# ufcg-lsd/custom-k8s-scheduler

Measured on AMD Instinct MI355X. Metric: pods scheduled/sec (exact sequential stream, 5,000 nodes x 100,000 pods), higher is better.
Workload: dtype int32+f64; 1 GPU; config2: 5,000 nodes x 100,000 pods, exact sequential, Fit+Balanced+QoS weights, percentageOfNodesToScore=100; engine=lookahead, launch=resident, table_layout=compact, lookahead=32, parallelism=single

## Files before the change

### custom-k8s-scheduler_amd/csrc/qs_ctx.hpp

```cpp
#pragma once
#include <hip/hip_runtime.h>
#include <rccl/rccl.h>

#include <mutex>
#include <string>
#include <vector>

#include "../../include/qsched.h"
#include "qs_device.hpp"
#include "qs_launch.hpp"

namespace qs_host {

constexpr int64_t kLimit = (1LL << 24) - 1;
constexpr int64_t kWideMemLimit = (1LL << 46) - 1;
constexpr int64_t kGrowLimit32 = (1LL << 31) - 1;
constexpr int64_t kGrowLimitF64 = (1LL << 53) - 1;
constexpr uint32_t kSoaMinNodes = 1u << 16;
constexpr uint32_t kAaMaxNodes = 1u << 20;

struct QsError {
    qs_status st;
    std::string msg;
};
// ... 66 lines not shown
    uint64_t epoch_after = 0;
    int shift = 0;
    bool wide = false;
    qs_ctx *owner = nullptr;
    hipGraphExec_t gexec = nullptr;
    std::vector<uint8_t> gkey;
    ~qs_stream() {
        if (gexec) (void)hipGraphExecDestroy(gexec);
    }
};

struct qs_ctx {
    std::mutex mu;
    uint64_t table_epoch = 0;
    qs_config cfg{};
    int device = 0;
    hipStream_t stream = nullptr;
    hipStream_t stream2 = nullptr;
    std::string err;
    qs_host::Mirror m;
    int shift = 20;
    bool wide = false;
    bool dev_valid = false;
    uint32_t zero_alloc = 0;
    qs::DevTable dt{};
    qs::DevCfg dc{};
    int32_t strat = 0;
    qs_host::DevBuf strat_tab;
    std::vector<qs_stream *> streams;
    qs_host::DevBuf tbl;
    qs_host::DevBuf soa;
    bool soa_valid = false;
    qs_host::DevBuf tbl_saved;
    qs_host::Mirror m_saved;
    bool saved = false;
    bool saved_wide = false;
    int saved_shift = 20;
    bool mirror_stale = false;
    uint64_t device_faults = 0;
    qs_host::DevBuf diag;
    qs_host::DevBuf scratch, lists, clists, dio, npart, normi, nstat, nfall, nrec, bctrl, one_pod, one_podx;
    qs_host::DevBuf vshard;
    void *pin = nullptr;
    size_t pin_bytes = 0;
    uint64_t score_seq = 0;
    qs_host::DevBuf score_gs;
    uint32_t pend = 0xFFFFFFFFu;
    qs_host::DevBuf hand;
    bool handoff_off = false;
    qs_host::DevBuf resctl;
    int res_timeouts = 0;
    bool res_cooldown = false;
    uint32_t inject_used = 0;
    bool last_resident = false;
    int32_t last_res_path = 0;
    int cus = 0;
    uint64_t run_seq = 0;
    bool last_waits = false;
    uint32_t cap = 0;
    int rank = 0, world = 1;
    ncclComm_t comm = nullptr;
    qs_host::DevBuf mbox, mbox_peers;
    std::vector<void *> mbox_opened;
    bool mbox_on = false;
    bool mbox_fine = false;
    bool mbox_broken = false;
    bool mbox_host = false;
    void *mbox_hptr = nullptr;
    std::string mbox_shm;
    std::vector<void *> mbox_hmaps;
};
namespace qs_host {
void mbox_host_release(qs_ctx *c);
}

namespace qs_host {
struct ShardPlan {
    uint32_t W, v0, nv;
};
inline ShardPlan shard_plan(const qs_ctx *c) {
    if (c->world > 1) return {(uint32_t)c->world, (uint32_t)c->rank, 1u};
    if (c->cfg.virtual_shards > 1) return {(uint32_t)c->cfg.virtual_shards, 0u, (uint32_t)c->cfg.virtual_shards};
    return {1u, 0u, 1u};
}
void exchange_lists(qs_ctx *c, uint64_t *lists, size_t per_rank_entries, hipStream_t stream);
void exchange_u32(qs_ctx *c, uint32_t *buf, size_t per_rank_words, hipStream_t stream);
void allreduce_max_u64(qs_ctx *c, uint64_t *buf, size_t count, hipStream_t stream);
void allreduce_max_u32(qs_ctx *c, uint32_t *buf, size_t count, hipStream_t stream);
constexpr size_t kDioWords = 68;
constexpr size_t kMbRanks = 16, kMbSlots = 3, kMbPartPerRank = 4096;
constexpr size_t kMbFlags = 2 * kMbRanks * 8;
constexpr size_t kMbListSlot = kMbRanks * 64 * 64 * 8;
constexpr size_t kMbPartSlot = kMbRanks * kMbPartPerRank * 16;
constexpr size_t kMbResSlots = 4, kMbResPods = 32;
constexpr size_t kMbResHello = kMbFlags + kMbSlots * (kMbListSlot + kMbPartSlot);
constexpr size_t kMbResFlags = kMbResHello + 256;
constexpr size_t kMbResLists = kMbResFlags + kMbResSlots * kMbResPods * kMbRanks * 8;
constexpr size_t kMbResNFlags = kMbResLists + kMbResSlots * kMbResPods * kMbRanks * 64 * 8;
constexpr size_t kMbResNorm = kMbResNFlags + kMbResSlots * kMbResPods * kMbRanks * 8;
constexpr size_t kMbBytes = kMbResNorm + kMbResSlots * kMbResPods * kMbRanks * 16;
inline uint64_t *mbox_lists(qs_ctx *c, uint32_t slot) {
    return reinterpret_cast<uint64_t *>(static_cast<char *>(c->mbox.p) + kMbFlags + slot * kMbListSlot);
}
inline uint4 *mbox_npart(qs_ctx *c, uint32_t slot) {
    return reinterpret_cast<uint4 *>(static_cast<char *>(c->mbox.p) + kMbFlags + kMbSlots * kMbListSlot +
                                     slot * kMbPartSlot);
// ... 6 lines not shown
```

### custom-k8s-scheduler_amd/csrc/qs_host.cpp

```cpp
#include "../../include/qsched.h"

#include <hip/hip_runtime.h>

#include <algorithm>
#include <atomic>
#include <chrono>
#include <cmath>
#include <cstddef>
#include <cstdio>
#include <cstdlib>
#include <cstring>
#include <exception>
#include <mutex>
#include <new>
#include <string>
#include <vector>
#include <functional>
#include <condition_variable>
#include <thread>

#include "qs_ctx.hpp"

using namespace qs;

using namespace qs_host;

namespace {

uint32_t feat_of(const qs_config &c) {
    uint32_t f = 0;
    if (c.enable_taint) f |= kFeatTaint;
    if (c.enable_affinity) f |= kFeatAffinity;
    return f;
}

void check_cfg(const qs_config &c) {
    if (c.abi_version != QS_ABI_VERSION) fail(QS_EINVAL, "qs_config.abi_version mismatch");
    if (c.fit_weight_cpu < 0 || c.fit_weight_mem < 0 || c.fit_weight_cpu > 65535 ||
        c.fit_weight_mem > 65535)
        fail(QS_EINVAL, "fit weights out of range");
    int64_t wmax = 0;
    for (int q = 0; q < 3; q++) {
        if (c.w_fit[q] < 0 || c.w_bal[q] < 0 || c.w_fit[q] > 65535 || c.w_bal[q] > 65535)
            fail(QS_EINVAL, "plugin weights must be in [0, 65535]");
        wmax = std::max<int64_t>(wmax, (int64_t)c.w_fit[q] + c.w_bal[q]);
    }
    if (c.w_taint < 0 || c.w_affinity < 0 || c.w_taint > 65535 || c.w_affinity > 65535)
        fail(QS_EINVAL, "plugin weights must be in [0, 65535]");
    if (c.n_fit_resources < 0 || c.n_fit_resources > QS_MAX_SCORE_RES)
        fail(QS_EINVAL, "n_fit_resources must be in [0, 4]");
    if (c.n_balanced_resources < 0 || c.n_balanced_resources > QS_MAX_SCORE_RES)
        fail(QS_EINVAL, "n_balanced_resources must be in [0, 4]");
    uint32_t seen = 0;
    for (int i = 0; i < c.n_fit_resources; i++) {
        const int32_t r = c.fit_resources[i].resource;
        if (r < QS_RES_CPU || r > QS_RES_EXT1) fail(QS_EINVAL, "fit_resources: unknown resource");
        if (seen & (1u << r)) fail(QS_EINVAL, "fit_resources: duplicate resource");
        seen |= 1u << r;
        if (c.fit_resources[i].weight < 1 || c.fit_resources[i].weight > 100)
            fail(QS_EINVAL, "fit_resources: weight must be in [1, 100]");
    }
    seen = 0;
    for (int i = 0; i < c.n_balanced_resources; i++) {
        const int32_t r = c.balanced_resources[i];
        if (r < QS_RES_CPU || r > QS_RES_EXT1) fail(QS_EINVAL, "balanced_resources: unknown resource");
        if (seen & (1u << r)) fail(QS_EINVAL, "balanced_resources: duplicate resource");
        seen |= 1u << r;
    }
    const int64_t tmax = 100 * (wmax + (c.enable_taint ? c.w_taint : 0) +
                                (c.enable_affinity ? c.w_affinity : 0));
    if (tmax >= 0x7FFFFFFF) fail(QS_EINVAL, "weighted total would overflow the packed key");
}

void fit_weights(const qs_config &c, int64_t w[5]) {
    for (int r = 0; r < 5; r++) w[r] = 0;
    if (c.n_fit_resources == 0) {
        w[QS_RES_CPU] = c.fit_weight_cpu;
        w[QS_RES_MEMORY] = c.fit_weight_mem;
        return;
    }
// ... 193 lines not shown
    for (uint32_t i = 0; i < n; i++) {
        const HostRow r = compact_row(c->m, i, c->shift, wide);
        if (wide) wrows[i] = to_drow_wide(r);
        else rows[i] = to_drow(r);
        masks[i] = DMask{r.th, r.ts, r.lb0, r.lb1};
        if (soa) {
            const int32_t f[kSCols] = {r.ac, r.am, r.rc, r.rm, r.zc, r.zm, r.np, r.mp, r.ae0, r.re0, r.ae1, r.re1};
            for (int k = 0; k < kSCols; k++) cols[(size_t)k * c->cap + i] = f[k];
        }
    }
    if (n) {
        if (wide) HIPCHK(hipMemcpyAsync(c->dt.wrows, wrows.data(), n * sizeof(DRowW), hipMemcpyHostToDevice, c->stream));
        else HIPCHK(hipMemcpyAsync(c->dt.rows, rows.data(), n * sizeof(DRow), hipMemcpyHostToDevice, c->stream));
        HIPCHK(hipMemcpyAsync(c->dt.masks, masks.data(), n * sizeof(DMask), hipMemcpyHostToDevice, c->stream));
        HIPCHK(hipMemcpyAsync(c->dt.zone, c->m.zone.data(), n * 4, hipMemcpyHostToDevice, c->stream));
    }
    if (c->dt.apps) {
        HIPCHK(hipMemsetAsync(c->dt.apps, 0, (size_t)kAppWords * c->cap * 4, c->stream));
        HIPCHK(hipMemsetAsync(c->dt.zcount, 0, (size_t)kMaxApps * kMaxZones * 4, c->stream));
    }
    if (soa) {
        c->soa.ensure(cols.size() * 4);
        for (int k = 0; k < kSCols; k++) c->dt.soa.c[k] = c->soa.as<int32_t>() + (size_t)k * c->cap;
        HIPCHK(hipMemcpyAsync(c->soa.p, cols.data(), cols.size() * 4, hipMemcpyHostToDevice, c->stream));
    }
    HIPCHK(hipStreamSynchronize(c->stream));
    c->dev_valid = true;
    c->soa_valid = soa;
    c->mirror_stale = false;
}

void ensure_soa(qs_ctx *c) {
    if (!c->dt.soa.c[0] || c->soa_valid) return;
    HIPCHK(launch_rows_to_soa(c->dt, c->stream));
    c->soa_valid = true;
}

void push_row(qs_ctx *c, uint32_t i, bool sync = true) {
    if (!c->dev_valid) return;
    const HostRow r = compact_row(c->m, i, c->shift, c->wide);
    hipLaunchKernelGGL(k_set_row, dim3(1), dim3(1), 0, c->stream, c->dt, i, r,
                       kFeatExt | kFeatTaint | kFeatAffinity);
    HIPCHK(hipGetLastError());
    if (sync) HIPCHK(hipStreamSynchronize(c->stream));
}

void flush_pending(qs_ctx *c) {
    if (c->pend == 0xFFFFFFFFu) return;
    const uint32_t i = c->pend;
    c->pend = 0xFFFFFFFFu;
    if (c->dev_valid && i < c->m.n) push_row(c, i, false);
}

void sync_mirror(qs_ctx *c) {
    if (!c->mirror_stale || !c->dev_valid) return;
    const uint32_t n = c->m.n;
    Mirror &m = c->m;
    if (c->wide) {
        std::vector<DRowW> rows(n);
        if (n) HIPCHK(hipMemcpyAsync(rows.data(), c->dt.wrows, n * sizeof(DRowW), hipMemcpyDeviceToHost, c->stream));
        HIPCHK(hipStreamSynchronize(c->stream));
        for (uint32_t i = 0; i < n; i++) {
            m.rc[i] = rows[i].rc;
            m.rm[i] = (int64_t)rows[i].rm;
            m.zc[i] = rows[i].zc;
            m.zm[i] = (int64_t)rows[i].zm;
            m.np[i] = rows[i].np;
            m.re[(size_t)i * QS_MAX_EXT] = rows[i].re0;
            m.re[(size_t)i * QS_MAX_EXT + 1] = rows[i].re1;
        }
    } else {
        std::vector<DRow> rows(n);
        if (n) HIPCHK(hipMemcpyAsync(rows.data(), c->dt.rows, n * sizeof(DRow), hipMemcpyDeviceToHost, c->stream));
        HIPCHK(hipStreamSynchronize(c->stream));
        for (uint32_t i = 0; i < n; i++) {
            m.rc[i] = rows[i].rc;
            m.rm[i] = (int64_t)rows[i].rm << c->shift;
            m.zc[i] = rows[i].zc;
            m.zm[i] = (int64_t)rows[i].zm << c->shift;
            m.np[i] = rows[i].np;
            m.re[(size_t)i * QS_MAX_EXT] = rows[i].re0;
            m.re[(size_t)i * QS_MAX_EXT + 1] = rows[i].re1;
        }
    }
    c->mirror_stale = false;
}

int pod_min_shift(const qs_pod &p) { return std::min(ctz64(p.req_mem), ctz64(p.nz_mem)); }

void check_pod(const qs_pod &p, uint32_t j) {
    auto bad = [&](const char *w) {
        fail(QS_EINVAL, std::string("pod ") + std::to_string(j) + ": " + w);
    };
    if (p.qos < 0 || p.qos > 2) bad("qos must be 0..2");
    if (p.req_cpu < 0 || p.req_mem < 0 || p.nz_cpu < 0 || p.nz_mem < 0) bad("negative request");
    for (int k = 0; k < QS_MAX_EXT; k++)
        if (p.req_ext[k] < 0 || p.req_ext[k] > kLimit) bad("req_ext out of range");
    if (p.req_cpu > kLimit || p.nz_cpu > kLimit) bad("cpu request out of range");
    if (p.req_mem > kWideMemLimit || p.nz_mem > kWideMemLimit) bad("memory request above 2^46 bytes");
    if (p.n_req_terms < 0 || p.n_req_terms > QS_MAX_TERMS || p.n_pref_terms < 0 ||
        p.n_pref_terms > QS_MAX_TERMS)
        bad("term count out of range");
    for (int t = 0; t < p.n_pref_terms; t++)
        if (p.pref_weight[t] < 0 || p.pref_weight[t] > 100) bad("preferred term weight must be 0..100");
    if (p.app < 0 || p.app >= QS_MAX_APPS) bad("app outside [0, QS_MAX_APPS)");
    if (p.anti_affinity < QS_AA_NONE || p.anti_affinity > QS_AA_ZONE) bad("anti_affinity must be 0..2");
}

uint32_t pod_flags(const qs_ctx *c, const qs_pod &p) {
    const uint32_t aff = c->cfg.enable_affinity ? 1u : 0u;
    return (uint32_t)p.qos | (aff * (uint32_t)p.n_req_terms << 4) | (aff * (uint32_t)p.n_pref_terms << 8) |
           ((uint32_t)p.anti_affinity << 12) | ((uint32_t)p.app << 16);
}

size_t pod_record_bytes(bool wide) { return wide ? sizeof(DPodW) : sizeof(DPod); }

void compact_pod(const qs_ctx *c, const qs_pod &p, uint32_t j, int shift, bool wide, void *dst) {
    check_pod(p, j);
    if (wide) {
        DPodW d{};
        d.rc = (int32_t)p.req_cpu;
        d.zc = (int32_t)p.nz_cpu;
        d.rm = (double)p.req_mem;
        d.zm = (double)p.nz_mem;
        d.re0 = (int32_t)p.req_ext[0];
        d.re1 = (int32_t)p.req_ext[1];
        d.wfit = (uint16_t)c->cfg.w_fit[p.qos];
// ... 362 lines not shown
    for (int q = 0; q < 3; q++) { cfg->w_fit[q] = wf[q]; cfg->w_bal[q] = wb[q]; }
    cfg->w_taint = 3;
    cfg->w_affinity = 2;
    cfg->qos_sort = 1;
}

qs_status qs_open(const qs_config *cfg, int device, qs_ctx **out) {
    g_open_err.clear();
    if (!cfg || !out) return open_failed(QS_EINVAL, "qs_open: null config or output pointer");
    *out = nullptr;
    qs_ctx *c = new (std::nothrow) qs_ctx();
    if (!c) return QS_ENOMEM;
    try {
        check_cfg(*cfg);
        c->cfg = *cfg;
        c->device = device;
        int ndev = 0;
        HIPCHK(hipGetDeviceCount(&ndev));
        if (device < 0 || device >= ndev) fail(QS_EINVAL, "no such device");
        HIPCHK(hipSetDevice(device));
        HIPCHK(hipStreamCreateWithFlags(&c->stream, hipStreamNonBlocking));
        HIPCHK(hipStreamCreateWithFlags(&c->stream2, hipStreamNonBlocking));
        c->dc = make_devcfg(c->cfg);
        c->scratch.ensure(scan_scratch_bytes());
        HIPCHK(hipMemset(c->scratch.p, 0, scan_scratch_bytes()));
    } catch (const QsError &e) {
        delete c;
        return open_failed(e.st, e.msg);
    } catch (...) {
        delete c;
        return open_failed(QS_EDEVICE, "qs_open: unexpected failure");
    }
    *out = c;
    return QS_OK;
}

qs_status qs_close(qs_ctx *c) {
    if (!c) return QS_EINVAL;
    {
        std::lock_guard<std::mutex> lk(c->mu);
        (void)hipSetDevice(c->device);
        if (c->stream) (void)hipStreamSynchronize(c->stream);
        if (c->comm) (void)ncclCommDestroy(c->comm);
        c->comm = nullptr;
        for (void *p : c->mbox_opened) (void)hipIpcCloseMemHandle(p);
        c->mbox_opened.clear();
        mbox_host_release(c);
        for (qs_stream *ps : c->streams) ps->owner = nullptr;
        c->streams.clear();
    }
    hipStream_t s = c->stream, s2 = c->stream2;
    if (s2) (void)hipStreamSynchronize(s2);
    if (c->pin) (void)hipHostFree(c->pin);
    delete c;
    if (s) (void)hipStreamDestroy(s);
    if (s2) (void)hipStreamDestroy(s2);
    return QS_OK;
}

static void shape_table(const qs_shape_point *sh, uint32_t n, uint8_t table[101]) {
    if (!sh || !table) fail(QS_EINVAL, "shape: null pointer");
    if (n < 1 || n > QS_MAX_SHAPE) fail(QS_EINVAL, "shape: 1 to 16 points");
    for (uint32_t i = 0; i < n; i++) {
        if (sh[i].utilization < 0 || sh[i].utilization > 100) fail(QS_EINVAL, "shape: utilization must be in [0, 100]");
        if (sh[i].score < 0 || sh[i].score > 10) fail(QS_EINVAL, "shape: score must be in [0, 10]");
        if (i && sh[i].utilization <= sh[i - 1].utilization)
            fail(QS_EINVAL, "shape: utilization must be strictly increasing");
    }
    for (int64_t p = 0; p <= 100; p++) {
        int64_t v = (int64_t)sh[n - 1].score * 10;
        for (uint32_t i = 0; i < n; i++) {
            if (p > sh[i].utilization) continue;
            const int64_t s1 = (int64_t)sh[i].score * 10;
            if (i == 0) { v = s1; break; }
            const int64_t s0 = (int64_t)sh[i - 1].score * 10, u0 = sh[i - 1].utilization, u1 = sh[i].utilization;
            v = s0 + (s1 - s0) * (p - u0) / (u1 - u0);
            break;
        }
        table[p] = (uint8_t)v;
    }
}

qs_status qs_shape_table(const qs_shape_point *shape, uint32_t n, uint8_t table[101]) {
    try {
        shape_table(shape, n, table);
    } catch (const QsError &) {
        return QS_EINVAL;
    }
    return QS_OK;
}

qs_status qs_set_scoring_strategy(qs_ctx *c, const qs_scoring_strategy *s) {
    return guarded(c, [&] {
        if (!s) fail(QS_EINVAL, "null scoring strategy");
        if (s->type != QS_STRATEGY_LEAST_ALLOCATED && s->type != QS_STRATEGY_MOST_ALLOCATED &&
            s->type != QS_STRATEGY_REQUESTED_TO_CAPACITY_RATIO)
            fail(QS_EINVAL, "unknown scoring strategy type");
        if (s->type != QS_STRATEGY_REQUESTED_TO_CAPACITY_RATIO && s->n_shape != 0)
            fail(QS_EINVAL, "a shape is given for a scoring strategy that takes none");
        alignas(16) uint8_t tab[128] = {0};
        if (s->type == QS_STRATEGY_REQUESTED_TO_CAPACITY_RATIO) {
            if (s->n_shape < 1 || s->n_shape > QS_MAX_SHAPE) fail(QS_EINVAL, "shape: 1 to 16 points");
            shape_table(s->shape, (uint32_t)s->n_shape, tab);
        } else {
            for (int p = 0; p <= 100; p++) tab[p] = (uint8_t)p;
        }
// ... 389 lines not shown
        if (g_sdiag && pk) score_diag_report(c->score_seq, std::chrono::steady_clock::now());
    }, true);
}

qs_status qs_stream_prepare(qs_ctx *c, const qs_pod *pods, uint32_t p, qs_stream **out) {
    if (!out) return QS_EINVAL;
    *out = nullptr;
    qs_stream *s = nullptr;
    qs_status st = guarded(c, [&] {
        if (p && !pods) fail(QS_EINVAL, "null pods");
        HIPCHK(hipSetDevice(c->device));
        s = new qs_stream();
        s->p = p;
        s->pods.assign(pods, pods + p);
        for (uint32_t j = 0; j < p; j++) check_pod(pods[j], j);
        ensure_layout(c, pods, p);
        s->shift = c->shift;
        s->wide = c->wide;
        s->feat = feat_of(c->cfg) | (c->wide ? kFeatWide | kFeatExt : 0u);
        bool has_ext = false;
        for (uint32_t j = 0; j < p && !has_ext; j++) has_ext = pods[j].req_ext[0] || pods[j].req_ext[1];
        if (has_ext) s->feat |= kFeatExt;
        s->feat |= res_feat(c->cfg, has_ext) | strat_feat(c);
        s->order = qos_order(pods, p, c->cfg.qos_sort != 0);
        const size_t rb = pod_record_bytes(c->wide);
        std::vector<uint8_t> dp(rb * std::max<uint32_t>(p, 1));
        const bool needx = feat_of(c->cfg) & (kFeatTaint | kFeatAffinity);
        std::vector<DPodX> dx(needx ? std::max<uint32_t>(p, 1) : 1);
        for (uint32_t k = 0; k < p; k++) {
            const uint32_t j = s->order[k];
            compact_pod(c, pods[j], j, c->shift, c->wide, dp.data() + rb * k);
            if (needx) dx[k] = compact_podx(c, pods[j]);
        }
        const size_t P1 = std::max<uint32_t>(p, 1);
        s->d_pods.ensure(rb * P1);
        s->d_podx.ensure(sizeof(DPodX) * dx.size());
        s->d_node.ensure(4 * P1);
        s->d_key.ensure(8 * P1);
        if (c->cfg.record_timestamps) s->d_stamp.ensure(8 * P1);
        HIPCHK(hipMemcpyAsync(s->d_pods.p, dp.data(), rb * p, hipMemcpyHostToDevice, c->stream));
        HIPCHK(hipMemcpyAsync(s->d_podx.p, dx.data(), sizeof(DPodX) * dx.size(), hipMemcpyHostToDevice, c->stream));
        HIPCHK(hipStreamSynchronize(c->stream));
        c->streams.push_back(s);
        s->owner = c;
    });
    if (st != QS_OK) {
        delete s;
        return st;
    }
    *out = s;
    return QS_OK;
}

qs_status qs_stream_run(qs_ctx *c, qs_stream *s, qs_mode mode, qs_stats *stats) {
    return guarded(c, [&] {
        if (!s) fail(QS_EINVAL, "null stream");
        if (mode != QS_MODE_EXACT && mode != QS_MODE_BATCHED) fail(QS_EINVAL, "unknown qs_mode");
        if (s->shift != c->shift || s->wide != c->wide) fail(QS_ESTATE, "node table re-laid out after prepare");
        HIPCHK(hipSetDevice(c->device));
        s->ran = false;
        s->mode_ran = -1;
        ++c->table_epoch;
        if (!c->dev_valid) upload_table(c);
        const uint32_t n = c->m.n, P = s->p;
        c->dc.feat = s->feat;
        const int eng = mode == QS_MODE_BATCHED ? QS_ENGINE_BATCHED : pick_engine(c, n);
        int32_t *on = s->d_node.as<int32_t>();
        uint64_t *ok = s->d_key.as<uint64_t>();
        uint64_t *st = c->cfg.record_timestamps ? s->d_stamp.as<uint64_t>() : nullptr;
        uint64_t batches = 0;
        hipEvent_t e0, e1;
        HIPCHK(hipEventCreate(&e0));
        HIPCHK(hipEventCreate(&e1));
        KernelTimer kt(c->cfg.profile_kernels != 0, c->stream, c->stream2);
        HIPCHK(hipEventRecord(e0, c->stream));
        if (P > 0 && n == 0) {
            HIPCHK(hipMemsetAsync(on, 0xFF, 4 * (size_t)P, c->stream));
            HIPCHK(hipMemsetAsync(ok, 0, 8 * (size_t)P, c->stream));
        } else if (P > 0) {
            const void *dp = s->d_pods.p;
            const DPodX *dx = s->d_podx.as<DPodX>();
            if (eng == QS_ENGINE_BATCHED) {
                batches = run_batched(c, s, dp, dx, on, ok, kt);
            } else if (eng == QS_ENGINE_PERSISTENT) {
                kt.begin(0, c->stream);
                HIPCHK(launch_persistent(c->dt, dp, dx, P, c->dc, on, ok, st, c->stream));
                kt.end(0, c->stream);
                batches = 1;
            } else if (eng == QS_ENGINE_SCAN) {
                HIPCHK(hipMemsetAsync(c->scratch.p, 0, scan_scratch_bytes(), c->stream));
                ensure_soa(c);
                for (uint32_t k = 0; k < P; k++) {
                    kt.begin(1, c->stream);
                    HIPCHK(launch_scan_pod(c->dt, dp, dx, k, c->dc, c->scratch.p, on, ok, st,
                                           nullptr, nullptr, nullptr, 1, c->stream));
                    kt.end(1, c->stream);
                    HIPCHK(launch_scan_pod(c->dt, dp, dx, k, c->dc, c->scratch.p, on, ok, st,
                                           nullptr, nullptr, nullptr, 2, c->stream));
                }
                batches = P;
            } else if (eng == QS_ENGINE_ALLREDUCE) {
                if (!c->comm)
                    fail(QS_ESTATE, "the all-reduce engine needs an RCCL communicator (qs_open_shard with an id)");
                const uint32_t V = c->world == 1 && c->cfg.virtual_shards > 1 ? (uint32_t)c->cfg.virtual_shards : 1u;
                const uint32_t R = V > 1 ? V : (uint32_t)c->world;
                DevTable dt = c->dt;
                std::memset(&dt.soa, 0, sizeof dt.soa);
                std::vector<uint32_t> sh(2 * (size_t)R);
                for (uint32_t r = 0; r < R; ++r) {
                    sh[2 * r] = (uint32_t)((uint64_t)n * r / R);
                    sh[2 * r + 1] = (uint32_t)((uint64_t)n * (r + 1) / R);
                }
                const uint32_t r0 = V > 1 ? 0u : (uint32_t)c->rank;
                c->vshard.ensure(8 * (size_t)R);
                HIPCHK(hipMemcpy(c->vshard.p, sh.data(), 8 * (size_t)R, hipMemcpyHostToDevice));
                HIPCHK(hipMemsetAsync(c->scratch.p, 0, scan_scratch_bytes(), c->stream));
                char *lohi = static_cast<char *>(c->scratch.p) + offsetof(ScanHead, lo);
                auto range = [&](uint32_t r) {
                    return hipMemcpyAsync(lohi, c->vshard.as<uint32_t>() + 2 * r, 8, hipMemcpyDeviceToDevice, c->stream);
                };
                if (V == 1) HIPCHK(range(r0));
                ScanHead *sc = c->scratch.as<ScanHead>();
                const bool norm = (c->dc.feat & (kFeatTaint | kFeatAffinity)) != 0;
                for (uint32_t k = 0; k < P; k++) {
                    kt.begin(1, c->stream);
                    if (norm) {
                        for (uint32_t v = 0; v < V; ++v) {
                            if (V > 1) HIPCHK(range(v));
// ... 130 lines not shown
                    constexpr int R = 4;
                    hipEvent_t esel[R], eres[R], est;
                    for (int r = 0; r < R; ++r) {
                        HIPCHK(hipEventCreateWithFlags(&esel[r], hipEventDisableTiming));
                        HIPCHK(hipEventCreateWithFlags(&eres[r], hipEventDisableTiming));
                    }
                    HIPCHK(hipEventCreateWithFlags(&est, hipEventDisableTiming));
                    HIPCHK(hipEventRecord(est, c->stream));
                    HIPCHK(hipStreamWaitEvent(c->stream2, est, 0));
                    select(0, c->stream2);
                    HIPCHK(hipEventRecord(esel[0], c->stream2));
                    for (uint32_t w = 0; w < nwin; ++w) {
                        if (w + 1 < nwin) {
                            if (w >= 1) HIPCHK(hipStreamWaitEvent(c->stream2, eres[(w - 1) % R], 0));
                            select(w + 1, c->stream2);
                            HIPCHK(hipEventRecord(esel[(w + 1) % R], c->stream2));
                        }
                        if (!handoff) HIPCHK(hipStreamWaitEvent(c->stream, esel[w % R], 0));
                        resolve(w);
                        HIPCHK(hipEventRecord(eres[w % R], c->stream));
                        if (sync_every && !capturing && (w + 1) % sync_every == 0) {
                            HIPCHK(hipStreamSynchronize(c->stream2));
                            HIPCHK(hipStreamSynchronize(c->stream));
                        }
                    }
                    hipEvent_t eend = nullptr;
                    if (handoff) {
                        HIPCHK(hipEventCreateWithFlags(&eend, hipEventDisableTiming));
                        HIPCHK(hipEventRecord(eend, c->stream2));
                        HIPCHK(hipStreamWaitEvent(c->stream, eend, 0));
                    }
                    for (int r = 0; r < R; ++r) {
                        (void)hipEventDestroy(esel[r]);
                        (void)hipEventDestroy(eres[r]);
                    }
                    (void)hipEventDestroy(est);
                    if (eend) (void)hipEventDestroy(eend);
                }
                };
                static const char *genv = getenv("QS_GRAPH");
                const bool graph_ok = !c->comm || (genv && genv[0] == '1');
                const bool use_graph = graph_ok && !handoff && !mbox && !kt.on && !diag_on && !(genv && genv[0] == '0');
                const char *renv = getenv("QS_RESIDENT");
                if (!c->cus) {
                    int cu = 0;
                    HIPCHK(hipDeviceGetAttribute(&cu, hipDeviceAttributeMultiprocessorCount, c->device));
                    c->cus = cu;
                }
                LaGeom pgeo = geo;
                if (norm && overlap && !(nw && nw[0] == '1')) pgeo.waves = 4;
                const char *rk = getenv("QS_RES_K32");
                if (rk && rk[0] == '0') pgeo.k32 = 0;
                LaGeom rgeo = la_stream_res_plan(pgeo, c->dc.feat, n, (uint32_t)c->cus, 2);
                if (rgeo.G > 0 && rgeo.K * rgeo.G + 1 > la_stream_res_max_blocks(rgeo, c->dc.feat, n, (uint32_t)c->cus))
                    rgeo = la_stream_res_plan(pgeo, c->dc.feat, n, (uint32_t)c->cus, 1);
                static const char *senv = getenv("QS_RES_SEL");
                uint32_t sel = rgeo.K * rgeo.G;
                if (senv && atoi(senv) > 0) sel = (uint32_t)atoi(senv);
                if (norm) sel = std::max(sel, rgeo.K * rgeo.G);
                const bool coresident =
                    rgeo.G > 0 && 1 + sel <= la_stream_res_max_blocks(rgeo, c->dc.feat, n, (uint32_t)c->cus);
                const bool res_transport = c->world == 1 ? !mbox && !c->comm : mbox;
                const bool res_allowed = c->res_timeouts < 2 && !c->res_cooldown;
                const bool resident = overlap && res_transport && res_allowed && !diag_on &&
                                      !(renv && renv[0] == '0') && rgeo.G > 0 && coresident;
                c->last_resident = resident;
                if (!resident) c->res_cooldown = false;
                if (resident) {
                    c->resctl.ensure(la_stream_res_ctl_bytes());
                    c->dc.ready = nullptr;
                    c->dc.epoch = 0;
                    c->dc.werr = reinterpret_cast<uint32_t *>(hw + 2);
                    c->last_waits = true;
                    HIPCHK(hipMemsetAsync(c->lists.p, 0, 8 * lwords * nbuf, c->stream));
                    HIPCHK(hipMemsetAsync(c->dio.p, 0, 2 * kDioWords * 4, c->stream));
                    HIPCHK(hipMemsetAsync(c->resctl.p, 0, la_stream_res_ctl_bytes(), c->stream));
                    HIPCHK(hipMemsetAsync(hw + 2, 0, 8, c->stream));
                    c->npart.ensure(16 * 2 * (size_t)rgeo.K * rgeo.G);
                    c->normi.ensure(16 * 2 * 64);
                    c->nstat.ensure(4 * 2 * 128 * (size_t)rgeo.K);
                    HIPCHK(hipMemsetAsync(c->nfall.p, 0, 16, c->stream));
                    const size_t rcw = std::max<size_t>(1, (size_t)rgeo.K * rgeo.G * rgeo.L);
                    c->clists.ensure(8 * rcw * 2);
                    ResShard rsh{1u, 0u, 0ull, nullptr, 0ull, 0ull, 0ull, 0ull, 0ull};
                    if (c->world > 1)
                        rsh = ResShard{(uint32_t)c->world, (uint32_t)c->rank, seq_run, c->mbox_peers.as<char *>(),
                                       kMbResHello, kMbResFlags, kMbResLists, kMbResNFlags, kMbResNorm};
                    DevCfg dcr = c->dc;
                    const char *inj = getenv("QS_INJECT_FAULT");
                    dcr.inject = (inject_once(c, "resident_stall", kInjResidentStall) ||
                                  (inj && std::strcmp(inj, "resident_stall_always") == 0)) ? 1u : 0u;
                    if (inj && std::strcmp(inj, "resident_skew") == 0) dcr.inject = 2u;
                    dcr.first_ticks = c->world > 1 ? 500000000ull : 0ull;
                    const char *fa = getenv("QS_FAST_ALLOC");
                    dcr.all_alloc = c->zero_alloc == 0 && !(fa && fa[0] == '0') ? 1u : 0u;
                    c->last_res_path = (!norm && rgeo.k32 ? 1 : 0) |
                                       (!norm && !(c->dc.feat & kFeatRes) && dcr.all_alloc ? 2 : 0);
                    static const bool rdiag_on = getenv("QS_RES_DIAG") && (getenv("QS_RES_DIAG")[0] == '1' ||
                                                                             getenv("QS_RES_DIAG")[0] == '2');
                    dcr.sel_diag = getenv("QS_RES_DIAG") && getenv("QS_RES_DIAG")[0] == '1' ? 1u : 0u;
                    uint64_t *rdiag = nullptr;
                    if (rdiag_on) {
                        c->diag.ensure(1024);
                        rdiag = c->diag.as<uint64_t>();
                        HIPCHK(hipMemsetAsync(rdiag, 0, 1024, c->stream));
                    }
                    kt.begin(3, c->stream);
                    HIPCHK(launch_la_stream_res(c->dt, dp, dx, dcr, P, rgeo, L0, c->clists.as<uint64_t>(),
                                                (uint32_t)lwords, (uint32_t)rcw, c->npart.as<uint4>(),
                                                c->normi.as<NormInfo>(), c->nstat.as<uint32_t>(),
                                                c->nfall.as<unsigned long long>(), on, ok,
                                                st, c->resctl.p, sel, rdiag, rsh, c->stream));
                    kt.end(3, c->stream);
                    if (rdiag) {
                        uint64_t h[128] = {0};
                        HIPCHK(hipMemcpyAsync(h, rdiag, 1024, hipMemcpyDeviceToHost, c->stream));
                        HIPCHK(hipStreamSynchronize(c->stream));
                        const double nw = h[3] ? (double)h[3] : 1.0;
                        fprintf(stderr, "QS_RES_DIAG resolver %.3f us per window; windows whose lists were not prefetched %llu of %llu (selectors %u)\n",
                                h[1] * 0.01 / nw, (unsigned long long)h[4], (unsigned long long)h[3], sel);
                        if (h[2])
                            fprintf(stderr, "QS_RES_DIAG selector 0: done seen %.2f us, its task finished %.2f us after "
                                            "the resolver's start of the window it overlaps (%llu windows)\n",
                                    h[13] * 0.01 / (double)h[2], h[14] * 0.01 / (double)h[2], (unsigned long long)h[2]);
                        {
                            std::vector<double> fin;
                            for (uint32_t k = 0; k < std::min(sel, 64u); ++k)
                                if (h[64 + k]) fin.push_back(h[64 + k] * 0.01);
                            std::sort(fin.begin(), fin.end());
                            if (!fin.empty()) {
                                fprintf(stderr, "QS_RES_DIAG selectors' mean finish (us after window start), sorted:");
                                for (double v : fin) fprintf(stderr, " %.1f", v);
                                fprintf(stderr, "\n");
                            }
                        }
                        if (h[36] + h[37] + h[38])
                            fprintf(stderr, "QS_RES_DIAG B3 -> B1 busy (ns per window, without the B1 wait): D %.0f, A %.0f, "
                                            "C %.0f\n", h[38] * 10.0 / nw, h[37] * 10.0 / nw, h[36] * 10.0 / nw);
                        if (h[33])
                            fprintf(stderr, "QS_RES_DIAG last list of a window published %.2f us after the start of "
                                            "the window before it (%llu windows; after 13 us %llu, after 15 us %llu)\n",
                                    h[32] * 0.01 / (double)h[33], (unsigned long long)h[33],
                                    (unsigned long long)h[34], (unsigned long long)h[35]);
                        if (h[6])
                            fprintf(stderr, "QS_RES_DIAG prefetch check: %llu windows short of lists, %.2f lists missing "
                                            "on average\n", (unsigned long long)h[6], (double)h[5] / (double)h[6]);
                        if (h[27] + h[28] + h[29] + h[30] + h[31])
                            fprintf(stderr, "QS_RES_DIAG window boundary (ns per window, wave D): bookkeeping %.0f "
                                            "-> B2 %.0f -> B3 %.0f -> B1 %.0f -> pod 0 decided %.0f\n",
                                    h[27] * 10.0 / nw, h[28] * 10.0 / nw, h[29] * 10.0 / nw, h[30] * 10.0 / nw,
                                    h[31] * 10.0 / nw);
                        if (h[19])
                            fprintf(stderr, "QS_RES_DIAG selector task (us): scoring %.2f chunk top-L %.2f publish/merge %.2f (tasks %llu, merges %llu)\n",
                                    h[16] * 0.01 / (double)h[19], h[17] * 0.01 / (double)h[19], h[18] * 0.01 / (double)h[19],
                                    (unsigned long long)h[19], (unsigned long long)h[20]);
                        if (h[12])
                            fprintf(stderr, "QS_RES_DIAG busy cycles/step: D %.0f A %.0f B %.0f C %.0f (steps %llu)\n",
                                    h[8] / (double)h[12], h[9] / (double)h[12], h[10] / (double)h[12],
                                    h[11] / (double)h[12], (unsigned long long)h[12]);
                        if (h[12])
                            fprintf(stderr, "QS_RES_DIAG step marks: D argmax %.0f | A pub+reads %.0f applied %.0f | C reads %.0f keyC %.0f loads %.0f\n",
                                    h[26] / (double)h[12], h[21] / (double)h[12], h[22] / (double)h[12],
                                    h[23] / (double)h[12], h[24] / (double)h[12], h[25] / (double)h[12]);
                    }
                } else if (use_graph) {
                    std::vector<uint8_t> key;
// ... 1 lines not shown
                        key.insert(key.end(), (const uint8_t *)p, (const uint8_t *)p + nb);
                    };
                    const void *ptrs[] = {c->dt.rows, c->dt.wrows, c->dt.masks, L0, C0, dio, st, (void *)c->comm, dp, dx,
                                          c->npart.p, c->normi.p, c->nfall.p};
                    put(ptrs, sizeof ptrs);
                    put(&c->dt.n, sizeof c->dt.n);
                    put(&c->dc, sizeof c->dc);
                    put(&geo, sizeof geo);
                    put(&overlap, sizeof overlap);
                    if (!s->gexec || s->gkey != key) {
                        if (s->gexec) (void)hipGraphExecDestroy(s->gexec);
                        s->gexec = nullptr;
                        HIPCHK(hipStreamBeginCapture(c->stream, hipStreamCaptureModeThreadLocal));
                        capturing = true;
                        try {
                            enqueue();
                        } catch (...) {
                            hipGraph_t g = nullptr;
                            (void)hipStreamEndCapture(c->stream, &g);
                            if (g) (void)hipGraphDestroy(g);
                            throw;
                        }
                        hipGraph_t g = nullptr;
                        HIPCHK(hipStreamEndCapture(c->stream, &g));
                        const hipError_t ie = hipGraphInstantiate(&s->gexec, g, nullptr, nullptr, 0);
                        (void)hipGraphDestroy(g);
                        HIPCHK(ie);
                        s->gkey = key;
                    }
                    HIPCHK(hipGraphLaunch(s->gexec, c->stream));
                } else {
                    enqueue();
                }
                batches = nwin;
                if (getenv("QS_HOSTTIME"))
                    fprintf(stderr, "QS_HOSTTIME enqueue %.3f ms for %u windows (overlap %d)\n",
                            std::chrono::duration<double>(std::chrono::steady_clock::now() - th0).count() * 1e3,
                            nwin, (int)overlap);
                if (diag_on) {
                    uint64_t h[16] = {0};
                    HIPCHK(hipMemcpyAsync(h, diag, 128, hipMemcpyDeviceToHost, c->stream));
                    HIPCHK(hipStreamSynchronize(c->stream));
                    const double np = h[5] ? (double)h[5] : 1.0;
                    fprintf(stderr, geo.waves == 1 ? "QS_DIAG resolve cycles/pod: cand %.0f issue %.0f fresh %.0f wmax %.0f commit %.0f (pods %llu, G=%u E=%u epl=%u)\n"
                                                   : "QS_DIAG resolve4 busy cycles/pod: D %.0f A %.0f B %.0f C %.0f (C row wait %.0f) (pods %llu, G=%u E=%u epl=%u)\n",
                            h[0] / np, h[1] / np, h[2] / np, h[3] / np, h[4] / np,
                            (unsigned long long)h[5], geo.G, geo.E, geo.epl);
                    if (geo.waves == 4)
                        fprintf(stderr, "QS_DIAG resolve4 pre-score cycles/pod: A %.0f C %.0f; per window: prologue %.0f epilogue %.0f\n",
                                h[6] / np, h[7] / np, h[8] / (double)nwin, h[9] / (double)nwin);
                }
            }
        }
        HIPCHK(hipEventRecord(e1, c->stream));
        HIPCHK(hipEventSynchronize(e1));
        float ms = 0.f;
        HIPCHK(hipEventElapsedTime(&ms, e0, e1));
        (void)hipEventDestroy(e0);
        (void)hipEventDestroy(e1);
        uint64_t rescans = 0, resumed = 0;
        if (eng == QS_ENGINE_LOOKAHEAD && c->last_waits) {
            uint64_t w = 0;
            HIPCHK(hipMemcpy(&w, c->hand.as<uint64_t>() + 2, 8, hipMemcpyDeviceToHost));
            if (inject_once(c, "handoff", kInjHandoff)) w = 1;
            if (w) {
                if (c->last_resident) {
                    ++c->res_timeouts;
                    c->res_cooldown = true;
                } else if (!c->mbox_on) {
                    c->handoff_off = true;
                }
                if (c->mbox_on && !c->comm) c->mbox_broken = true;
                fail(QS_ETIMEOUT, c->mbox_on ? "mailbox exchange timed out (a peer never posted its window)"
                                             : c->last_resident
                                                   ? "resident lookahead stream timed out (a hand-off never arrived); "
                                                     "the next run uses per-window launches"
                                                   : "lookahead window hand-off timed out (lists never published); "
                                                     "the context falls back to stream events");
            }
        }
        if (eng == QS_ENGINE_LOOKAHEAD && c->last_resident) c->res_timeouts = 0;
        if (eng == QS_ENGINE_LOOKAHEAD && c->nfall.p) {
            uint64_t h[2] = {0, 0};
            HIPCHK(hipMemcpy(h, c->nfall.p, 16, hipMemcpyDeviceToHost));
            rescans = h[0];
            resumed = h[1];
            if (getenv("QS_NORM_DIAG"))
                fprintf(stderr, "QS_NORM_DIAG rescans %llu resumed windows %llu\n", (unsigned long long)h[0],
                        (unsigned long long)h[1]);
        }
        c->mirror_stale = true;
        if (eng != QS_ENGINE_SCAN) c->soa_valid = false;
        kt.finish();
        maybe_inject_fault(c, "stream_run");
        sync_mirror(c);
        s->ran = true;
        s->mode_ran = (int)mode;
        s->epoch_after = ++c->table_epoch;
        if (stats) {
            std::memset(stats, 0, sizeof(*stats));
            for (int k = 0; k < 4; k++) {
                stats->kernel_s[k] = kt.secs[k];
                stats->kernel_launches[k] = kt.count[k];
            }
            stats->pods = P;
            stats->evals = (uint64_t)P * n;
            stats->wall_s = ms * 1e-3;
            stats->batches = batches;
            stats->truncations = rescans;
            stats->engine_used = eng;
            stats->table_layout = c->wide ? 1 : 0;
            stats->resumed_windows = resumed;
            stats->resident = (eng == QS_ENGINE_LOOKAHEAD && c->last_resident) ? 1 : 0;
            stats->resident_path = stats->resident ? c->last_res_path : 0;
            stats->device_faults = c->device_faults;
        }
    });
}

qs_status qs_stream_results(qs_ctx *c, qs_stream *s, int32_t *placement, uint64_t *best_key) {
    return guarded(c, [&] {
        if (!s || !s->ran) fail(QS_ESTATE, "stream has not run");
        HIPCHK(hipSetDevice(c->device));
        const uint32_t P = s->p;
        std::vector<int32_t> node(P);
        std::vector<uint64_t> key(P);
        if (P) {
            HIPCHK(hipMemcpyAsync(node.data(), s->d_node.p, 4 * (size_t)P, hipMemcpyDeviceToHost, c->stream));
            HIPCHK(hipMemcpyAsync(key.data(), s->d_key.p, 8 * (size_t)P, hipMemcpyDeviceToHost, c->stream));
            HIPCHK(hipStreamSynchronize(c->stream));
        }
        for (uint32_t k = 0; k < P; k++) {
            const uint32_t j = s->order[k];
            if (placement) placement[j] = node[k];
            if (best_key) best_key[j] = key[k];
        }
    });
}

qs_status qs_stream_free(qs_ctx *c, qs_stream *s) {
    (void)c;
    if (s && s->owner) {
        std::lock_guard<std::mutex> lk(s->owner->mu);
        auto &v = s->owner->streams;
        v.erase(std::remove(v.begin(), v.end(), s), v.end());
    }
    delete s;
    return QS_OK;
}

qs_status qs_table_save(qs_ctx *c) {
    return guarded(c, [&] {
        if (!c->dev_valid) fail(QS_ESTATE, "no node table loaded");
        HIPCHK(hipSetDevice(c->device));
        sync_mirror(c);
        c->tbl_saved.ensure(c->tbl.bytes);
        HIPCHK(hipMemcpyAsync(c->tbl_saved.p, c->tbl.p, c->tbl.bytes, hipMemcpyDeviceToDevice, c->stream));
        HIPCHK(hipStreamSynchronize(c->stream));
        c->m_saved = c->m;
        c->saved_wide = c->wide;
        c->saved_shift = c->shift;
        c->saved = true;
    });
}

qs_status qs_table_restore(qs_ctx *c) {
    return guarded(c, [&] {
        if (!c->saved || !c->dev_valid || c->tbl_saved.bytes != c->tbl.bytes || c->saved_wide != c->wide ||
            c->saved_shift != c->shift)
            fail(QS_ESTATE, "no matching qs_table_save snapshot");
        HIPCHK(hipSetDevice(c->device));
        HIPCHK(hipMemcpyAsync(c->tbl.p, c->tbl_saved.p, c->tbl.bytes, hipMemcpyDeviceToDevice, c->stream));
        c->m = c->m_saved;
        c->zero_alloc = count_zero_alloc(c->m);
        c->mirror_stale = false;
        ++c->table_epoch;
        c->soa_valid = false;
    });
}

qs_status qs_schedule_stream(qs_ctx *c, const qs_pod *pods, uint32_t p, qs_mode mode,
                             int32_t *placement, qs_stats *stats) {
    using clk = std::chrono::steady_clock;
    auto t0 = clk::now();
    qs_stream *s = nullptr;
    qs_status st = qs_stream_prepare(c, pods, p, &s);
    if (st != QS_OK) return st;
    auto t1 = clk::now();
    qs_stats local{};
    st = qs_stream_run(c, s, mode, &local);
    if (st != QS_OK) { qs_stream_free(nullptr, s); return st; }
    auto t2 = clk::now();
    st = qs_stream_results(c, s, placement, nullptr);
    if (st == QS_OK && c->cfg.record_timestamps && p > 1) {
        std::vector<uint64_t> stamps(p);
        if (hipMemcpy(stamps.data(), s->d_stamp.p, 8 * (size_t)p, hipMemcpyDeviceToHost) == hipSuccess)
            percentile_stats(stamps, &local);
    }
    auto t3 = clk::now();
    for (uint32_t j = 0; j < p && st == QS_OK; j++) {
        if (placement[j] >= 0) local.placed++;
        else local.unschedulable++;
    }
    qs_status st2 = qs_stream_free(c, s);
    if (st == QS_OK) st = st2;
    local.h2d_s = std::chrono::duration<double>(t1 - t0).count();
    local.d2h_s = std::chrono::duration<double>(t3 - t2).count();
    if (stats) *stats = local;
    return st;
}

size_t qs_struct_size(int which) {
    switch (which) {
        case 0: return sizeof(qs_config);
        case 1: return sizeof(qs_node_soa);
        case 2: return sizeof(qs_node_row);
        case 3: return sizeof(qs_pod);
        case 4: return sizeof(qs_container);
        case 5: return sizeof(qs_stats);
        case 6: return sizeof(qs_scoring_strategy);
        default: return 0;
    }
}

static qs_status fit_errors(qs_ctx *c, qs_stream *s, const uint32_t *pods, uint32_t mreq, uint32_t *counts,
                            uint32_t *tcounts) {
    return guarded(c, [&] {
// ... 86 lines not shown
```

Baseline: 2.223 million pods/s.

## Cut host overhead around stream runs: reuse events, pinned staging, batched readbacks

Events are now created once per context and reused, and a pinned host staging buffer is added. The end-of-run readbacks of the nfall counters, the hand-off error word and the node-table rows are enqueued asynchronously into that buffer and waited on with one stream sync, replacing several blocking hipMemcpy calls and a pageable vector copy. The resident-kernel occupancy query is cached per geometry, one dio memset is dropped, and restore reuses a zero-alloc count saved at snapshot time. An optional QS_HOSTTIME phase timer is also added. The gain is limited to fixed per-call host latency, and it adds pinned memory and cache state that must stay consistent.

```diff
diff --git a/custom-k8s-scheduler_amd/csrc/qs_ctx.hpp b/custom-k8s-scheduler_amd/csrc/qs_ctx.hpp
--- a/custom-k8s-scheduler_amd/csrc/qs_ctx.hpp
+++ b/custom-k8s-scheduler_amd/csrc/qs_ctx.hpp
@@ -142,6 +142,14 @@
     int res_timeouts = 0;
     bool res_cooldown = false;
     uint32_t inject_used = 0;
+    hipEvent_t ev0 = nullptr, ev1 = nullptr;
+    void *stage = nullptr;
+    size_t stage_bytes = 0;
+    struct ResOcc {
+        uint32_t feat, n, E, e2, k32, cus, blocks;
+    };
+    std::vector<ResOcc> res_occ;
+    uint32_t saved_zero_alloc = 0;
     bool last_resident = false;
     int32_t last_res_path = 0;
     int cus = 0;
diff --git a/custom-k8s-scheduler_amd/csrc/qs_host.cpp b/custom-k8s-scheduler_amd/csrc/qs_host.cpp
--- a/custom-k8s-scheduler_amd/csrc/qs_host.cpp
+++ b/custom-k8s-scheduler_amd/csrc/qs_host.cpp
@@ -26,6 +26,30 @@
 using namespace qs_host;
 
 namespace {
+
+struct HostPhases {
+    enum { kSetup, kPlan, kMemsets, kLaunch, kWait, kReads, kMirror, kCount };
+    bool on;
+    double us[kCount] = {0, 0, 0, 0, 0, 0, 0};
+    std::chrono::steady_clock::time_point last;
+    HostPhases() : on(getenv("QS_HOSTTIME") != nullptr) {
+        if (on) last = std::chrono::steady_clock::now();
+    }
+    void mark(int ph) {
+        if (!on) return;
+        const auto t = std::chrono::steady_clock::now();
+        us[ph] += std::chrono::duration<double>(t - last).count() * 1e6;
+        last = t;
+    }
+    void print_run() const {
+        if (!on) return;
+        double tot = 0;
+        for (double v : us) tot += v;
+        fprintf(stderr, "QS_HOSTTIME run (us): setup %.1f plan %.1f memsets %.1f launch %.1f wait %.1f "
+                        "reads %.1f mirror %.1f total %.1f\n",
+                us[kSetup], us[kPlan], us[kMemsets], us[kLaunch], us[kWait], us[kReads], us[kMirror], tot);
+    }
+};
 
 uint32_t feat_of(const qs_config &c) {
     uint32_t f = 0;
@@ -325,14 +349,36 @@
     if (c->dev_valid && i < c->m.n) push_row(c, i, false);
 }
 
-void sync_mirror(qs_ctx *c) {
+constexpr size_t kStageRows = 64;
+void ensure_stage(qs_ctx *c, size_t bytes) {
+    if (bytes <= c->stage_bytes) return;
+    if (c->stage) (void)hipHostFree(c->stage);
+    c->stage = nullptr;
+    c->stage_bytes = 0;
+    HIPCHK(hipHostMalloc(&c->stage, bytes, hipHostMallocDefault));
+    c->stage_bytes = bytes;
+}
+size_t table_row_bytes(const qs_ctx *c) { return c->wide ? sizeof(DRowW) : sizeof(DRow); }
+
+void stage_rows(qs_ctx *c) {
+    const size_t nb = (size_t)c->m.n * table_row_bytes(c);
+    ensure_stage(c, kStageRows + nb);
+    if (!nb) return;
+    const void *src = c->wide ? (const void *)c->dt.wrows : (const void *)c->dt.rows;
+    HIPCHK(hipMemcpyAsync(static_cast<char *>(c->stage) + kStageRows, src, nb, hipMemcpyDeviceToHost, c->stream));
+}
+
+void sync_mirror(qs_ctx *c, bool staged = false) {
     if (!c->mirror_stale || !c->dev_valid) return;
     const uint32_t n = c->m.n;
     Mirror &m = c->m;
+    if (!staged) {
+        stage_rows(c);
+        HIPCHK(hipStreamSynchronize(c->stream));
+    }
+    const char *base = static_cast<const char *>(c->stage) + kStageRows;
     if (c->wide) {
-        std::vector<DRowW> rows(n);
-        if (n) HIPCHK(hipMemcpyAsync(rows.data(), c->dt.wrows, n * sizeof(DRowW), hipMemcpyDeviceToHost, c->stream));
-        HIPCHK(hipStreamSynchronize(c->stream));
+        const DRowW *rows = reinterpret_cast<const DRowW *>(base);
         for (uint32_t i = 0; i < n; i++) {
             m.rc[i] = rows[i].rc;
             m.rm[i] = (int64_t)rows[i].rm;
@@ -343,9 +389,7 @@
             m.re[(size_t)i * QS_MAX_EXT + 1] = rows[i].re1;
         }
     } else {
-        std::vector<DRow> rows(n);
-        if (n) HIPCHK(hipMemcpyAsync(rows.data(), c->dt.rows, n * sizeof(DRow), hipMemcpyDeviceToHost, c->stream));
-        HIPCHK(hipStreamSynchronize(c->stream));
+        const DRow *rows = reinterpret_cast<const DRow *>(base);
         for (uint32_t i = 0; i < n; i++) {
             m.rc[i] = rows[i].rc;
             m.rm[i] = (int64_t)rows[i].rm << c->shift;
@@ -814,6 +858,9 @@
     hipStream_t s = c->stream, s2 = c->stream2;
     if (s2) (void)hipStreamSynchronize(s2);
     if (c->pin) (void)hipHostFree(c->pin);
+    if (c->stage) (void)hipHostFree(c->stage);
+    if (c->ev0) (void)hipEventDestroy(c->ev0);
+    if (c->ev1) (void)hipEventDestroy(c->ev1);
     delete c;
     if (s) (void)hipStreamDestroy(s);
     if (s2) (void)hipStreamDestroy(s2);
@@ -1309,11 +1356,22 @@
     return QS_OK;
 }
 
+static uint32_t res_max_blocks(qs_ctx *c, const LaGeom &g, uint32_t n) {
+    const uint32_t feat = c->dc.feat, cus = (uint32_t)c->cus;
+    for (const qs_ctx::ResOcc &o : c->res_occ)
+        if (o.feat == feat && o.n == n && o.E == g.E && o.e2 == g.e2 && o.k32 == g.k32 && o.cus == cus) return o.blocks;
+    const uint32_t blocks = la_stream_res_max_blocks(g, feat, n, cus);
+    if (c->res_occ.size() >= 64) c->res_occ.clear();
+    c->res_occ.push_back({feat, n, g.E, g.e2, g.k32, cus, blocks});
+    return blocks;
+}
+
 qs_status qs_stream_run(qs_ctx *c, qs_stream *s, qs_mode mode, qs_stats *stats) {
     return guarded(c, [&] {
         if (!s) fail(QS_EINVAL, "null stream");
         if (mode != QS_MODE_EXACT && mode != QS_MODE_BATCHED) fail(QS_EINVAL, "unknown qs_mode");
         if (s->shift != c->shift || s->wide != c->wide) fail(QS_ESTATE, "node table re-laid out after prepare");
+        HostPhases hp;
         HIPCHK(hipSetDevice(c->device));
         s->ran = false;
         s->mode_ran = -1;
@@ -1326,11 +1384,13 @@
         uint64_t *ok = s->d_key.as<uint64_t>();
         uint64_t *st = c->cfg.record_timestamps ? s->d_stamp.as<uint64_t>() : nullptr;
         uint64_t batches = 0;
-        hipEvent_t e0, e1;
-        HIPCHK(hipEventCreate(&e0));
-        HIPCHK(hipEventCreate(&e1));
+        if (!c->ev0) HIPCHK(hipEventCreate(&c->ev0));
+        if (!c->ev1) HIPCHK(hipEventCreate(&c->ev1));
+        const hipEvent_t e0 = c->ev0, e1 = c->ev1;
+        const void *rd_werr = nullptr, *rd_nfall = nullptr;
         KernelTimer kt(c->cfg.profile_kernels != 0, c->stream, c->stream2);
         HIPCHK(hipEventRecord(e0, c->stream));
+        hp.mark(HostPhases::kSetup);
         if (P > 0 && n == 0) {
             HIPCHK(hipMemsetAsync(on, 0xFF, 4 * (size_t)P, c->stream));
             HIPCHK(hipMemsetAsync(ok, 0, 8 * (size_t)P, c->stream));
@@ -1567,34 +1627,37 @@
                 const char *rk = getenv("QS_RES_K32");
                 if (rk && rk[0] == '0') pgeo.k32 = 0;
                 LaGeom rgeo = la_stream_res_plan(pgeo, c->dc.feat, n, (uint32_t)c->cus, 2);
-                if (rgeo.G > 0 && rgeo.K * rgeo.G + 1 > la_stream_res_max_blocks(rgeo, c->dc.feat, n, (uint32_t)c->cus))
+                if (rgeo.G > 0 && rgeo.K * rgeo.G + 1 > res_max_blocks(c, rgeo, n))
                     rgeo = la_stream_res_plan(pgeo, c->dc.feat, n, (uint32_t)c->cus, 1);
                 static const char *senv = getenv("QS_RES_SEL");
                 uint32_t sel = rgeo.K * rgeo.G;
                 if (senv && atoi(senv) > 0) sel = (uint32_t)atoi(senv);
                 if (norm) sel = std::max(sel, rgeo.K * rgeo.G);
                 const bool coresident =
-                    rgeo.G > 0 && 1 + sel <= la_stream_res_max_blocks(rgeo, c->dc.feat, n, (uint32_t)c->cus);
+                    rgeo.G > 0 && 1 + sel <= res_max_blocks(c, rgeo, n);
                 const bool res_transport = c->world == 1 ? !mbox && !c->comm : mbox;
                 const bool res_allowed = c->res_timeouts < 2 && !c->res_cooldown;
                 const bool resident = overlap && res_transport && res_allowed && !diag_on &&
                                       !(renv && renv[0] == '0') && rgeo.G > 0 && coresident;
                 c->last_resident = resident;
+                hp.mark(HostPhases::kPlan);
                 if (!resident) c->res_cooldown = false;
+                rd_werr = c->last_waits ? hw + 2 : nullptr;
+                rd_nfall = c->nfall.p;
                 if (resident) {
                     c->resctl.ensure(la_stream_res_ctl_bytes());
+                    rd_werr = hw + 2;
                     c->dc.ready = nullptr;
                     c->dc.epoch = 0;
                     c->dc.werr = reinterpret_cast<uint32_t *>(hw + 2);
                     c->last_waits = true;
                     HIPCHK(hipMemsetAsync(c->lists.p, 0, 8 * lwords * nbuf, c->stream));
-                    HIPCHK(hipMemsetAsync(c->dio.p, 0, 2 * kDioWords * 4, c->stream));
                     HIPCHK(hipMemsetAsync(c->resctl.p, 0, la_stream_res_ctl_bytes(), c->stream));
                     HIPCHK(hipMemsetAsync(hw + 2, 0, 8, c->stream));
+                    HIPCHK(hipMemsetAsync(c->nfall.p, 0, 16, c->stream));
                     c->npart.ensure(16 * 2 * (size_t)rgeo.K * rgeo.G);
                     c->normi.ensure(16 * 2 * 64);
                     c->nstat.ensure(4 * 2 * 128 * (size_t)rgeo.K);
-                    HIPCHK(hipMemsetAsync(c->nfall.p, 0, 16, c->stream));
                     const size_t rcw = std::max<size_t>(1, (size_t)rgeo.K * rgeo.G * rgeo.L);
                     c->clists.ensure(8 * rcw * 2);
                     ResShard rsh{1u, 0u, 0ull, nullptr, 0ull, 0ull, 0ull, 0ull, 0ull};
@@ -1620,6 +1683,7 @@
                         rdiag = c->diag.as<uint64_t>();
                         HIPCHK(hipMemsetAsync(rdiag, 0, 1024, c->stream));
                     }
+                    hp.mark(HostPhases::kMemsets);
                     kt.begin(3, c->stream);
                     HIPCHK(launch_la_stream_res(c->dt, dp, dx, dcr, P, rgeo, L0, c->clists.as<uint64_t>(),
                                                 (uint32_t)lwords, (uint32_t)rcw, c->npart.as<uint4>(),
@@ -1627,6 +1691,7 @@
                                                 c->nfall.as<unsigned long long>(), on, ok,
                                                 st, c->resctl.p, sel, rdiag, rsh, c->stream));
                     kt.end(3, c->stream);
+                    hp.mark(HostPhases::kLaunch);
                     if (rdiag) {
                         uint64_t h[128] = {0};
                         HIPCHK(hipMemcpyAsync(h, rdiag, 1024, hipMemcpyDeviceToHost, c->stream));
@@ -1734,16 +1799,25 @@
                 }
             }
         }
+        hp.mark(HostPhases::kLaunch);
         HIPCHK(hipEventRecord(e1, c->stream));
-        HIPCHK(hipEventSynchronize(e1));
+        ensure_stage(c, kStageRows + (size_t)n * table_row_bytes(c));
+        uint64_t *hres = static_cast<uint64_t *>(c->stage);
+        hres[0] = hres[1] = hres[2] = 0;
+        if (rd_nfall && rd_werr == static_cast<const char *>(rd_nfall) + 16) {
+            HIPCHK(hipMemcpyAsync(hres, rd_nfall, 24, hipMemcpyDeviceToHost, c->stream));
+        } else {
+            if (rd_nfall) HIPCHK(hipMemcpyAsync(hres, rd_nfall, 16, hipMemcpyDeviceToHost, c->stream));
+            if (rd_werr) HIPCHK(hipMemcpyAsync(hres + 2, rd_werr, 8, hipMemcpyDeviceToHost, c->stream));
+        }
+        stage_rows(c);
+        HIPCHK(hipStreamSynchronize(c->stream));
+        hp.mark(HostPhases::kWait);
         float ms = 0.f;
         HIPCHK(hipEventElapsedTime(&ms, e0, e1));
-        (void)hipEventDestroy(e0);
-        (void)hipEventDestroy(e1);
         uint64_t rescans = 0, resumed = 0;
         if (eng == QS_ENGINE_LOOKAHEAD && c->last_waits) {
-            uint64_t w = 0;
-            HIPCHK(hipMemcpy(&w, c->hand.as<uint64_t>() + 2, 8, hipMemcpyDeviceToHost));
+            uint64_t w = hres[2];
             if (inject_once(c, "handoff", kInjHandoff)) w = 1;
             if (w) {
                 if (c->last_resident) {
@@ -1762,20 +1836,22 @@
             }
         }
         if (eng == QS_ENGINE_LOOKAHEAD && c->last_resident) c->res_timeouts = 0;
-        if (eng == QS_ENGINE_LOOKAHEAD && c->nfall.p) {
-            uint64_t h[2] = {0, 0};
-            HIPCHK(hipMemcpy(h, c->nfall.p, 16, hipMemcpyDeviceToHost));
+        if (eng == QS_ENGINE_LOOKAHEAD && rd_nfall) {
+            const uint64_t h[2] = {hres[0], hres[1]};
             rescans = h[0];
             resumed = h[1];
             if (getenv("QS_NORM_DIAG"))
                 fprintf(stderr, "QS_NORM_DIAG rescans %llu resumed windows %llu\n", (unsigned long long)h[0],
                         (unsigned long long)h[1]);
         }
+        hp.mark(HostPhases::kReads);
         c->mirror_stale = true;
         if (eng != QS_ENGINE_SCAN) c->soa_valid = false;
         kt.finish();
         maybe_inject_fault(c, "stream_run");
-        sync_mirror(c);
+        sync_mirror(c, true);
+        hp.mark(HostPhases::kMirror);
+        hp.print_run();
         s->ran = true;
         s->mode_ran = (int)mode;
         s->epoch_after = ++c->table_epoch;
@@ -1840,6 +1916,7 @@
         HIPCHK(hipMemcpyAsync(c->tbl_saved.p, c->tbl.p, c->tbl.bytes, hipMemcpyDeviceToDevice, c->stream));
         HIPCHK(hipStreamSynchronize(c->stream));
         c->m_saved = c->m;
+        c->saved_zero_alloc = count_zero_alloc(c->m);
         c->saved_wide = c->wide;
         c->saved_shift = c->shift;
         c->saved = true;
@@ -1851,10 +1928,17 @@
         if (!c->saved || !c->dev_valid || c->tbl_saved.bytes != c->tbl.bytes || c->saved_wide != c->wide ||
             c->saved_shift != c->shift)
             fail(QS_ESTATE, "no matching qs_table_save snapshot");
+        HostPhases hp;
         HIPCHK(hipSetDevice(c->device));
         HIPCHK(hipMemcpyAsync(c->tbl.p, c->tbl_saved.p, c->tbl.bytes, hipMemcpyDeviceToDevice, c->stream));
+        hp.mark(0);
         c->m = c->m_saved;
-        c->zero_alloc = count_zero_alloc(c->m);
+        hp.mark(1);
+        c->zero_alloc = c->saved_zero_alloc;
+        hp.mark(2);
+        if (hp.on)
+            fprintf(stderr, "QS_HOSTTIME restore (us): device copy enqueue %.1f mirror copy %.1f zero-alloc count %.1f\n",
+                    hp.us[0], hp.us[1], hp.us[2]);
         c->mirror_stale = false;
         ++c->table_epoch;
         c->soa_valid = false;
```

Result: no change. 2.219 million pods/s (-0.2%).
